# onecodex/finch-rs

Hardware: AMD Instinct MI355X
Metric: bases/sec sketched (k=21, n=1000) (higher is better)
Workload: dtype u64; 1 GPU; 50.0 Gbase synthetic 150 bp reads in total (BASELINE configs[3]), split into 1 contiguous read block (one per GPU), mash k=21 n=1000 seed 0, blocks resident in HBM as packed stream, partial sketches merged on the host; reads_per_gpu=333333334, reads_total=333333334, parallelism=read-block sharding x1, host merge; one process, one GPU

## Files before the change

finch_rs_amd/csrc/build.py:

```python
#!/usr/bin/env python3
import os
import subprocess
import sys
from concurrent.futures import ThreadPoolExecutor

HERE = os.path.dirname(os.path.abspath(__file__))
PKG = os.path.dirname(HERE)
OUT = os.path.join(PKG, "libfinch_hip.so")
OBJ = os.path.join(HERE, "obj")
NPARTS = 4
HIPCC = os.environ.get("HIPCC", "/opt/rocm/bin/hipcc")
FLAGS = ["--offload-arch=gfx950", "-O3", "-std=c++17", "-fPIC", "-Wall", "-Wno-unused-function", "-Wno-cuda-compat"]
FLAGS += os.environ.get("FH_EXTRA_FLAGS", "").split()
K2_FLAGS = ["-mllvm", "-amdgpu-sched-strategy=max-ilp", "-mllvm", "-pragma-unroll-threshold=200000"]
if "FH_K2_FLAGS" in os.environ:
    K2_FLAGS = os.environ["FH_K2_FLAGS"].split()
K2S_FLAGS_LAST = ["-mllvm", "-amdgpu-sched-strategy=iterative-ilp", "-mllvm", "-pragma-unroll-threshold=200000"]
if "FH_K2S_FLAGS_LAST" in os.environ:
    K2S_FLAGS_LAST = os.environ["FH_K2S_FLAGS_LAST"].split()
elif "FH_K2_FLAGS" in os.environ:
    K2S_FLAGS_LAST = K2_FLAGS
if "FH_OUT" in os.environ:
    OUT = os.environ["FH_OUT"]
    OBJ = os.path.join(HERE, "obj", "ab_" + os.path.splitext(os.path.basename(OUT))[0])

K2WS_FLAGS = os.environ["FH_K2WS_FLAGS"].split() if "FH_K2WS_FLAGS" in os.environ else ["-mllvm", "-amdgpu-sched-strategy=max-ilp"]
K2W_FLAGS = os.environ["FH_K2W_FLAGS"].split() if "FH_K2W_FLAGS" in os.environ else ["-mllvm", "-amdgpu-sched-strategy=max-ilp"]
SOURCES = ["fh_core.h", "fh_device.h", "fh_kernels.h", "fh_k2_common.h", "fh_k2_lds.h", "fh_internal.h", "fh_options.h", "fh_options.cpp", "fh_k2b.hip", "fh_k2bw.hip", "fh_batch.hip", "fh_batch_plan.h", "fh_batch_large.hip", "fh_records.hip", "fh_records_plan.h", "fh_screen.hip", "fh_screen.h", "fh_epilogue_dev.h", "fh_k2w.hip", "fh_k2.hip", "fh_k2s.hip", "fh_k2ws.hip", "fh_kernels.hip", "fh_big.hip", "fh_text.hip", "fh_bgzf.hip", "fh_api.hip", "fh_dist.hip", "fh_dist.h", "fh_dist_dev.h", "fh_index.hip", "fh_index.h", "fh_cluster.h", "fh_merge_path.h", "fh_gather.hip", "fh_matrix.hip", "fh_matrix.h", "fh_moments.hip", "fh_moments.h", "fh_merge_lib.hip", "fh_merge_lib.h", "fh_counts.hip", "fh_counts.h", "fh_host.cpp", "fh_library.cpp",
           "fh_host_model.h", "fh_inflate.h", "fh_pargz.h", "fh_slot_pipe.h", "fh_entries.h", "fh_serial.cpp", os.path.join("..", "..", "include", "finch_host.h"),
           os.path.join("..", "..", "include", "finch_hip.h")]


def _newest_src():
    return max(os.path.getmtime(os.path.join(HERE, s)) for s in SOURCES)


def _run(cmd):
    r = subprocess.run(cmd, cwd=HERE, stdout=subprocess.PIPE, stderr=subprocess.STDOUT, text=True)
    if r.returncode != 0:
        raise RuntimeError("command failed: %s\n%s" % (" ".join(cmd), r.stdout))
    return r.stdout


# ... 90 lines not shown
```

finch_rs_amd/csrc/fh_api.hip:

```cpp
#include <hip/hip_runtime.h>
#include <sched.h>

#include <algorithm>
#include <atomic>
#include <chrono>
#include <cmath>
#include <cstdarg>
#include <cstdio>
#include <cstdlib>
#include <cstring>
#include <condition_variable>
#include <mutex>
#include <string>
#include <thread>
#include <vector>

#include "../../include/finch_hip.h"
#include "fh_core.h"
#include "fh_counts.h"
#include "fh_strip.h"
#include "fh_device.h"
#include "fh_kernels.h"
#include "fh_internal.h"
#include "fh_options.h"

using namespace fh;

namespace {

thread_local std::string g_err;

int fail(int code, const char *fmt, ...) {
    char buf[512];
    va_list ap;
    va_start(ap, fmt);
    vsnprintf(buf, sizeof buf, fmt, ap);
    va_end(ap);
    g_err = buf;
    return code;
// ... 116 lines not shown
    } spec;
    uint64_t n_fast_finish = 0, n_spec_deferred = 0, n_spec_recovered = 0;
    uint32_t epi_pending = 0, epi_units = 0;
    uint8_t *proc_buf = nullptr;
    uint64_t proc_cap = 0, proc_fill = 0, proc_total_bases = 0;
    bool proc_continuing = false, proc_in_record = false, proc_in_cut = false;
    bool device_clean = false;
    uint64_t final_text_bases = 0;
    uint32_t *left_buf[2] = {nullptr, nullptr};
    uint32_t seg_hint = 0, blk_seg = 0, blk_sub = 1;
    uint64_t gran = TILE_POS;
    uint32_t *h_probe = nullptr;
    bool probe_seen = false;
    hipEvent_t probe_ev = nullptr;
    uint32_t probe_answer = 0;
    uint32_t probe_breakers = 0;
    uint64_t n_seg_launches = 0, n_seg_probes = 0;
    uint64_t max_waves = 0;
    uint64_t max_range = 0;
    uint64_t tau_lo = 0;
    bool no_spec = false;
    uint64_t n_spec = 0, n_spec_fallback = 0, n_spec_rescaled = 0;
    uint32_t *smp_list = nullptr, *smp_hist = nullptr, *h_smp_hist = nullptr;
    uint64_t smp_list_cap = 0;
    uint64_t n_sampled = 0;
    uint64_t ins_seen = 0;
    double novelty = 1.0;
    uint64_t n_launches = 0, n_relaunches = 0;
    uint8_t *h_stage[N_STAGE] = {nullptr, nullptr};
    uint8_t *d_stage[N_STAGE] = {nullptr, nullptr};
// ... 207 lines not shown
    if (s->open_loop) {
        P = ((remaining + G - 1) / G) * G;
    } else {
        const double room = (double)s->live_target - (double)std::min<uint64_t>(s->last_live, s->live_target);
        const double fr = fill_rate(s);
        double p = fr > 0.0 ? (s->big_mode ? 1.0 : 0.5) * room / fr : 1e19;
        P = p >= 1e18 ? remaining + G : (uint64_t)p;
    }
    if (s->max_range) P = std::min<uint64_t>(P, s->max_range);
    P = std::max<uint64_t>((P / G) * G, G);
    return std::min<uint64_t>(P, ((remaining + G - 1) / G) * G);
}

int check_ctl(fh_sketcher *s);
int flush_epilogue(fh_sketcher *s);
int recover_spec(fh_sketcher *s);
int reread_above(fh_sketcher *s, const uint8_t *seq, uint64_t len, uint64_t base_pos, uint64_t p_begin, uint64_t p_end, uint64_t lo);
int sketch_positions(fh_sketcher *s, const uint8_t *d_seq, uint64_t len, uint64_t base_pos, uint64_t pos, uint64_t n_pos, uint64_t lo_end);
int big_prune(fh_sketcher *s, bool sorted = true);
int grow_table(fh_sketcher *s, uint64_t new_live_cap);

int collect_profile(fh_sketcher *s) {
    for (size_t i = 0; i < s->prof_used; ++i) {
        float ms = 0.f;
        HIP_TRY(hipEventElapsedTime(&ms, s->prof_events[i].first, s->prof_events[i].second));
        s->prof_ms += ms;
    }
    s->prof_used = 0;
    return FH_OK;
}
// ... 161 lines not shown
    r.seq = d_seq;
    r.len = len;
    r.base_pos = base_pos;
    r.p_begin = pos;
    r.p_end = end;
    r.seg = (s->blk_seg && (s->p.k > 32 || (!s->p.hash_mask && !s->tau_lo)) && pos % s->gran == 0) ? s->blk_seg : 0u;
    r.seg_sub = r.seg ? s->blk_sub : 1u;
    const uint64_t tile = r.seg ? (uint64_t)seg_tile_pos(r.seg, r.seg_sub) : (uint64_t)TILE_POS;
    const uint64_t tiles = (end - pos + tile - 1) / tile;
    if (tiles >= (1ull << 31)) return fail(FH_ERR_INVALID, "block too large for one range");
    r.tiles_total = (uint32_t)tiles;
    static const uint32_t unit_knob = [] {
        const char *e = cfg("unit_tiles");
        return e ? (uint32_t)atoi(e) : 0u;
    }();
    r.unit_tiles = unit_knob ? unit_knob : (tiles < (uint64_t)UNIT_TILES * 2 * s->max_waves ? 1u : (uint32_t)UNIT_TILES);
    r.max_units = MAX_UNITS;
    if (r.seg) {
        static const uint32_t seg_pull = [] {
            const char *e = cfg("seg_pull_pos");
            return e ? (uint32_t)atoi(e) : (uint32_t)MAX_UNITS * UNIT_TILES * TILE_POS;
        }();
        if (!unit_knob) r.unit_tiles = 1u;
        r.max_units = std::max<uint32_t>(1u, seg_pull / (uint32_t)(tile * r.unit_tiles));
    }
    r.n_units = (uint32_t)((tiles + r.unit_tiles - 1) / r.unit_tiles);
    r.n_left_in = 0;
    r.left_cur = 0;
    r.gated = gated;
    r.verdict = spec_tau != 0;
    r.admit_at_start = admit_rate(s->last_tau);
// ... 11 lines not shown
    HIP_TRY(launch_queue_reset(s->ctl, 1u, soft_limit_of(s), read_first_of(s), s->stream, spec_tau != 0, spec_tau, gated, first_total));
    if (int rc = launch_pending(s)) return rc;
    r.active = true;
    if (s->profiling) s->prof_positions += end - pos;
    s->dirty = true;
    return FH_OK;
}

int set_tau(fh_sketcher *s, uint64_t tau) {
    if (int rc = flush_epilogue(s)) return rc;
    HIP_TRY(launch_set_tau(s->ctl, tau, s->stream));
    s->last_tau = tau;
    return FH_OK;
}

constexpr uint64_t SPEC_MAX_POS = 64ull << 20, SPEC_PREFIX_POS = 32ull << 20;
int speculative_first_block(fh_sketcher *s, const uint8_t *d_seq, uint64_t len, uint64_t base_pos, uint64_t n_pos,
                            bool *done) {
    *done = false;
    const double want = 4.0 * (double)std::max<uint64_t>(s->p.size, 1);
    if (s->no_spec || s->max_range || s->p.hash_mask || n_pos < 32768 || n_pos > SPEC_MAX_POS ||
        want * 2.0 >= (double)n_pos)
        return FH_OK;
    if (s->p.kind == FH_KIND_SCALED && s->p.size == 0) return FH_OK;
    uint64_t tau_spec = (uint64_t)(want / (double)n_pos * 18446744073709551616.0);
    if (s->p.kind == FH_KIND_SCALED) tau_spec = std::max(tau_spec, s->max_hash);
    if (tau_spec == 0 || tau_spec >= EMPTY64 - 1) return FH_OK;
    if (s->fast && !s->big_mode && s->p.kind == FH_KIND_MASH && s->p.size > 0) {
        s->n_spec++;
        s->n_spec_deferred++;
        const bool was_open = s->open_loop;
// ... 222 lines not shown
            s->prof_used++;
        }
        HIP_TRY(launch_ac_count((int)s->p.k, a, s->stream));
        if (e1) {
            HIP_TRY(hipEventRecord(e1, s->stream));
            s->prof_launches++;
            s->prof_positions += a.p_end - a.p_begin;
        }
        s->n_launches++;
    }
    s->positions_done += n_pos;
    s->ac_dirty = true;
    return FH_OK;
}

int sketch_device_range(fh_sketcher *s, const uint8_t *d_seq, uint64_t len, uint64_t base_pos) {
    if (int rc = drain(s)) return rc;
    if (len < s->p.k) return FH_OK;
    if (s->p.kind == FH_KIND_ALL_COUNTS) return ac_count_block(s, d_seq, len);
    const uint64_t n_pos = len - s->p.k + 1;
    s->blk_seg = 0;
    s->blk_sub = 1;
    s->gran = TILE_POS;
    bool probe_behind = false;
    {
        static const bool seg_off = cfg("no_seg") != nullptr;
        static const uint64_t probe_min = [] {
            const char *e = cfg("seg_probe_min");
            return e ? strtoull(e, nullptr, 10) : (16ull << 20);
        }();
        static const uint64_t probe_wait_min = [] {
// ... 45 lines not shown
    struct ProbeBehind {
        fh_sketcher *s;
        const uint8_t *seq;
        uint64_t len;
        bool on;
        ~ProbeBehind() {
            if (!on || !s->h_probe) return;
            if (launch_seg_probe(seq, len, s->h_probe, s->stream) == hipSuccess) {
                if (!s->probe_ev && hipEventCreateWithFlags(&s->probe_ev, hipEventDisableTiming) != hipSuccess) s->probe_ev = nullptr;
                if (s->probe_ev) (void)hipEventRecord(s->probe_ev, s->stream);
                s->probe_seen = true;
                s->n_seg_probes++;
            }
        }
    } probe_guard{s, d_seq, len, probe_behind};
    uint64_t pos = 0;
    uint64_t lo_end = 0;
    bool sampled = false;
    if (s->positions_done == 0 && s->tau_lo == 0) {
        bool done = false;
        if (int rc = sampled_first_block(s, d_seq, len, base_pos, n_pos, &sampled, &done)) return rc;
        if (sampled && done) return FH_OK;
        if (sampled) lo_end = n_pos;
    }
    if (!sampled && s->positions_done == 0 && s->tau_lo == 0) {
        static const uint64_t prefix_pos = cfg("spec_prefix_pos") ? std::max<uint64_t>(1ull << 20, strtoull(cfg("spec_prefix_pos"), nullptr, 10)) : SPEC_PREFIX_POS;
        const uint64_t spec_pos = n_pos <= SPEC_MAX_POS ? n_pos : std::max<uint64_t>(prefix_pos / s->gran, 1) * s->gran;
        bool done = false;
        if (int rc = speculative_first_block(s, d_seq, len, base_pos, spec_pos, &done)) return rc;
        if (done) {
            if (spec_pos == n_pos) return FH_OK;
            pos = spec_pos;
        } else if (s->tau_lo) {
            if (int rc = reread_above(s, d_seq, len, base_pos, 0, spec_pos, s->tau_lo)) return rc;
            if (spec_pos == n_pos) return FH_OK;
            pos = spec_pos;
        }
    }
    return sketch_positions(s, d_seq, len, base_pos, pos, n_pos, lo_end);
}

int sketch_positions(fh_sketcher *s, const uint8_t *d_seq, uint64_t len, uint64_t base_pos, uint64_t pos, uint64_t n_pos, uint64_t lo_end) {
// ... 78 lines not shown
    if ((uint64_t)s->last_live >= s->p.size) {
        s->positions_done += sp.n_pos;
    } else {
        s->n_spec_fallback++;
        if (int rc = reread_above(s, sp.range.seq, sp.range.len, sp.range.base_pos, sp.range.p_begin, sp.range.p_end, sp.tau)) return rc;
    }
    if (queued.active)
        if (int rc = sketch_positions(s, queued.seq, queued.len, queued.base_pos, queued.p_begin, queued.p_end, 0)) return rc;
    return FH_OK;
}

int check_ctl(fh_sketcher *s) {
    if (int rc = flush_epilogue(s)) return rc;
    HIP_TRY(hipMemcpyAsync(s->h_ctl, s->ctl, sizeof(Ctl), hipMemcpyDeviceToHost, s->stream));
    HIP_TRY(hipStreamSynchronize(s->stream));
    if (s->h_ctl->overflow == 1) return fail(FH_ERR_CAPACITY, "device hash table capacity exceeded");
    if (s->h_ctl->overflow == 2) return fail(FH_ERR_CAPACITY, "hash collision log capacity exceeded");
    return FH_OK;
}

int ensure_big_buffers(fh_sketcher *s, uint32_t M) {
    if (M <= s->big_cap) return FH_OK;
    HIP_TRY(hipStreamSynchronize(s->stream));
    if (s->keys_a) { (void)hipFree(s->keys_a); (void)hipFree(s->keys_b); (void)hipFree(s->slots_a); (void)hipFree(s->slots_b); (void)hipFree(s->sort_tmp); }
    s->keys_a = s->keys_b = nullptr; s->slots_a = s->slots_b = nullptr; s->sort_tmp = nullptr;
    const uint32_t cap = (uint32_t)std::min<uint64_t>((uint64_t)M + M / 2 + 1024, s->live_cap);
    HIP_TRY(dev_malloc(&s->keys_a, (size_t)cap * 8));
    HIP_TRY(dev_malloc(&s->keys_b, (size_t)cap * 8));
    HIP_TRY(dev_malloc(&s->slots_a, (size_t)cap * 4));
    HIP_TRY(dev_malloc(&s->slots_b, (size_t)cap * 4));
// ... 491 lines not shown
        uint64_t held = handle_bytes(s);
        for (const fh_sketcher *q : g_pool) held += handle_bytes(q);
        if (g_pool.size() < pool_max() && held <= pool_max_bytes()) {
            g_pool.push_back(s);
            return;
        }
    }
    destroy_handle(s);
}

namespace {
void destroy_handle(fh_sketcher *s) {
    if (!s) return;
    (void)hipSetDevice(s->device);
    if (s->stream) (void)hipStreamSynchronize(s->stream);
    for (auto &pe : s->prof_events) {
        (void)hipEventDestroy(pe.first);
        (void)hipEventDestroy(pe.second);
    }
    for (int i = 0; i < N_STAGE; ++i) {
        if (s->h_stage[i]) (void)hipHostFree(s->h_stage[i]);
        if (s->d_stage[i]) (void)hipFree(s->d_stage[i]);
        if (s->stage_done[i]) (void)hipEventDestroy(s->stage_done[i]);
        (void)hipFree(s->d_packed[i]);
        (void)hipFree(s->d_blk_a[i]);
        (void)hipFree(s->d_blk_b[i]);
    }
    (void)hipFree(s->d_text_tot);
    (void)hipFree(s->d_lines);
    for (int q = 0; q < fh_sketcher::BZ_STREAMS; ++q) {
// ... 52 lines not shown
    if (s->h_smp_hist) (void)hipHostFree(s->h_smp_hist);
    if (s->h_probe) (void)hipHostFree(s->h_probe);
    if (s->probe_ev) (void)hipEventDestroy(s->probe_ev);
    if (s->copy_stream) {
        (void)hipStreamSynchronize(s->copy_stream);
        (void)hipStreamDestroy(s->copy_stream);
    }
    if (s->stream) (void)hipStreamDestroy(s->stream);
    delete s;
}
}

int fh_reset(fh_sketcher *s) {
    if (!s) return fail(FH_ERR_INVALID, "null handle");
    if (int rc = set_device(s)) return rc;
    gzip_quiesce(s);
    if (s->ac_table && (s->ac_dirty || s->ac_check)) {
        const uint64_t bins = ac_bins((int)s->p.k);
        HIP_TRY(hipMemsetAsync(s->ac_table, 0, bins * 4, s->stream));
        HIP_TRY(hipMemsetAsync(s->ac_sat, 0, std::max<uint64_t>(bins / 8, 4), s->stream));
    }
    s->ac_dirty = s->ac_check = false;
    s->ac_windows = 0;
    if (s->device_clean && s->finished && !s->pend.active && !s->epi_pending) {
        s->device_clean = false;
        return init_state(s, false);
    }
    s->device_clean = false;
    if (s->spec.pending && !s->pend.active) s->spec.pending = false;
    if (int rc = drain(s)) return rc;
// ... 129 lines not shown
    if (!s) return fail(FH_ERR_INVALID, "null argument");
    if (launches) *launches = s->n_seg_launches;
    if (probes) *probes = s->n_seg_probes;
    if (stride) *stride = s->blk_seg;
    return FH_OK;
}

int fh_push_device(fh_sketcher *s, const void *dev_bytes, uint64_t len) {
    if (!s || (!dev_bytes && len)) return fail(FH_ERR_INVALID, "null argument");
    if (s->finished) return fail(FH_ERR_STATE, "sketcher already finished; call fh_reset");
    if (int rc = proc_flush(s)) return rc;
    if (((uintptr_t)dev_bytes & 15u) != 0) return fail(FH_ERR_INVALID, "device block must be 16-byte aligned");
    if (int rc = set_device(s)) return rc;
    s->carry_len = 0;
    s->dprev_len = 0;
    int rc = sketch_device_range(s, (const uint8_t *)dev_bytes, len, s->stream_off);
    s->stream_off += len;
    return rc;
}

static uint64_t strip_block(uint8_t *dst, const uint8_t *src, uint64_t n) {
    static const unsigned cap = [] {
        const char *e = cfg("host_threads");
        const unsigned v = e ? (unsigned)atoi(e) : 8u;
        return v ? v : 1u;
    }();
    const unsigned hw = std::max(1u, std::thread::hardware_concurrency());
    const size_t nt = std::min<size_t>(std::min<size_t>(hw, cap), n >> 21);
    if (nt <= 1) return fh_strip::strip(dst, src, n);
    const size_t per = (n + nt - 1) / nt;
    std::vector<size_t> kept(nt + 1, 0);
    auto lo_of = [&](size_t t) { return std::min<size_t>(n, t * per); };
// ... 729 lines not shown
        *total_bases = s->final_text_bases;
        return FH_OK;
    }
    if (int rc = set_device(s)) return rc;
    if (int rc = drain(s)) return rc;
    if (int rc = check_ctl(s)) return rc;
    *total_bases = s->h_ctl->text_bases;
    return FH_OK;
}

int fh_push_block(fh_sketcher *s, const uint8_t *bytes, uint64_t len) { return fh_push_block_ex(s, bytes, len, 0u); }

int fh_sync(fh_sketcher *s) {
    if (!s) return fail(FH_ERR_INVALID, "null handle");
    if (int rc = set_device(s)) return rc;
    if (int rc = proc_flush(s)) return rc;
    if (int rc = drain(s)) return rc;
    if (int rc = check_ctl(s)) return rc;
    return collect_profile(s);
}

static size_t result_count(const fh_sketcher *s) { return s->res_built ? s->res.size() : s->r_n; }

static int ensure_wide(fh_sketcher *s) {
    if (!s->wide_pending) return FH_OK;
    if (int rc = set_device(s)) return rc;
    const size_t n = s->r_n;
    HIP_TRY(hipMemcpyAsync(s->r_hash, s->o_hash, n * 8ull, hipMemcpyDeviceToHost, s->stream));
    HIP_TRY(hipMemcpyAsync(s->r_kmer, s->o_kmer, n * 8ull, hipMemcpyDeviceToHost, s->stream));
    if (s->r_kmer_hi) HIP_TRY(hipMemcpyAsync(s->r_kmer_hi, s->o_kmer_hi, n * 8ull, hipMemcpyDeviceToHost, s->stream));
// ... 73 lines not shown
        HIP_TRY(dev_malloc(&tmp, bytes));
        HIP_TRY(hipMemcpyPeerAsync(tmp, dst->device, src->ac_table, src->device, bytes, dst->stream));
        from = tmp;
    }
    hipError_t e = launch_ac_add(dst->ac_table, from, ac_bins((int)dst->p.k), dst->stream);
    if (e == hipSuccess) e = hipStreamSynchronize(dst->stream);
    (void)hipFree(tmp);
    if (e != hipSuccess) return fail(FH_ERR_HIP, "fh_merge (AllCounts): %s", hipGetErrorString(e));
    dst->ac_check = dst->ac_dirty = true;
    return ac_finish(dst);
}

int fh_finish(fh_sketcher *s, uint64_t *n_out, uint64_t *total_kmers) {
    if (!s) return fail(FH_ERR_INVALID, "null handle");
    if (int rc = set_device(s)) return rc;
    if (s->p.kind == FH_KIND_ALL_COUNTS) {
        if (!s->finished) {
            if (int rc = proc_flush(s)) return rc;
            if (int rc = ac_finish(s)) return rc;
        }
        if (n_out) *n_out = s->r_n;
        if (total_kmers) *total_kmers = s->total_kmers;
        return FH_OK;
    }
    static const bool trace = cfg("trace") != nullptr;
    auto now = [] { return std::chrono::steady_clock::now(); };
    auto ms = [](std::chrono::steady_clock::time_point a, std::chrono::steady_clock::time_point b) {
        return std::chrono::duration<double, std::milli>(b - a).count();
    };
    const auto t0 = now();
// ... 16 lines not shown
            if (int rc = ensure_out(s, (uint32_t)std::min<uint64_t>(s->p.size + 1, SMALL_MAX))) return rc;
            if (int rc = ensure_h_out(s->out_stride * (wide ? 40 : 32) + 64)) return rc;
            static const bool no_fold = cfg("no_reset_fold") != nullptr;
            EpiArgs e = epi_args(s, s->epi_pending | EPI_PRUNE_FORCE | EPI_SORT | EPI_GATHER | (s->spec.pending ? EPI_NEED_SPEC : 0u) |
                                        (no_fold ? 0u : EPI_RESET));
            e.n_units = s->epi_units;
            s->epi_pending = 0;
            e.check_units = s->pend.active ? s->pend.n_units : 0u;
            e.tau0 = initial_tau(s);
            e.hist_on = s->hist ? 1u : 0u;
            e.out = (uint64_t *)s->h_out;
            e.out_stride = (uint32_t)s->out_stride;
            e.h_ctl = s->h_ctl;
            HIP_TRY(launch_small_epilogue(e, s->stream));
            HIP_TRY(hipStreamSynchronize(s->stream));
            const Ctl &c = *s->h_ctl;
            if (c.overflow == 1) return fail(FH_ERR_CAPACITY, "device hash table capacity exceeded");
            if (c.overflow == 2) return fail(FH_ERR_CAPACITY, "hash collision log capacity exceeded");
            fused = c.sorted == FIN_OK || c.sorted == FIN_OK_RESET;
            s->device_clean = c.sorted == FIN_OK_RESET;
            if (fused) {
                s->spec.pending = false;
                s->pend.active = false;
                s->last_tau = c.tau;
                s->last_live = c.n_live;
                s->ins_seen = c.inserted_total;
                s->n_fast_finish++;
            }
        }
        if (!fused) {
// ... 702 lines not shown
```

finch_rs_amd/csrc/fh_kernels.hip:

```cpp
#include <hip/hip_runtime.h>

#include <atomic>

#include "fh_core.h"
#include "fh_device.h"
#include "fh_epilogue_dev.h"
#include "fh_kernels.h"

namespace fh {

hipError_t launch_k2(int k, const SketchArgs &a, int blocks, hipStream_t st) {
    static_assert(FH_NPARTS == 4, "dispatcher below is written for 4 parts");
    if (k < 1 || k > FH_MAX_K) return hipErrorInvalidValue;
    if (k > 32 && a.seg_stride) {
        if (!seg_launch_ok((uint32_t)k, a.seg_stride, a.seg_sub)) return hipErrorInvalidValue;
        switch ((k - 33) / (32 / FH_NPARTS)) {
        case 0: return launch_k2ws_part0(k, a, st);
        case 1: return launch_k2ws_part1(k, a, st);
        case 2: return launch_k2ws_part2(k, a, st);
        default: return launch_k2ws_part3(k, a, st);
        }
    }
    if (k > 32) {
        switch ((k - 33) / (32 / FH_NPARTS)) {
// ... 140 lines not shown
        const u64 key = keys[i];
        if (((u32)(key >> shift) & 2047u) == bin) list[atomicAdd(&wsum[0], 1u)] = key;
    }
    __syncthreads();
    const u32 want = rank - below - 1u;
    if (tid < in_bin) {
        const u64 mine = list[tid];
        u32 smaller = 0;
        for (u32 j = 0; j < in_bin; ++j) smaller += list[j] < mine ? 1u : 0u;
        if (smaller == want) bcast[0] = mine;
    }
    __syncthreads();
    const u64 r = bcast[0];
    __syncthreads();
    return r;
}

struct SmallLds {
    u64 *keys;
    u64 *skeys;
    u32 *sslots;
    u32 *hist;
    u32 *wsum;
    u64 *bcast;
    u32 *cnt;
};
constexpr size_t SMALL_LDS_BYTES = (size_t)SMALL_MAX * 8 + (size_t)SMALL_SORT_MAX * 12;
constexpr u32 PRUNE_DECLINED = 0xFFFFFFFFu;

__device__ __forceinline__ void sort_wide_dev(u32 *live, u32 *scratch, u32 M, const SmallLds L) {
// ... 45 lines not shown
    u64 *keys = L.keys;
    constexpr int PER = SMALL_MAX / 1024;
    u32 my_slot[PER];
#pragma unroll
    for (int j = 0; j < PER; ++j) {
        const u32 i = tid + (u32)j * 1024u;
        my_slot[j] = 0u;
        if (i < M) {
            const u32 sl = live[i];
            my_slot[j] = sl;
            keys[i] = table[sl].hash;
        }
    }
    if (tid < 2) L.cnt[tid] = 0;
    __syncthreads();
    u64 tau;
    u32 keep;
    if (kind == 0u) {
        if ((u64)M >= size && size > 0) {
            tau = lds_select_kth_fast(keys, M, (u32)size, L.hist, L.wsum, L.bcast, reinterpret_cast<unsigned char *>(L.skeys));
            keep = (u32)size;
        } else if (size == 0) {
            tau = 0ull;
            keep = 0;
        } else {
            tau = EMPTY64;
            keep = M;
        }
    } else {
        u32 c = 0;
// ... 19 lines not shown
    if (sort_out && keep > (u32)SMALL_SORT_MAX) {
        const u32 nd_now = ctl->n_dead;
        if (!keep_all || keep != M || nd_now > dead_cap || M > dead_cap - nd_now) {
            if (tid == 0) ctl->need_big = 1u;
            return PRUNE_DECLINED;
        }
        sort_wide_dev(live, dead + nd_now, M, L);
        if (tid == 0) {
            ctl->n_live = keep;
            const u64 cur = ctl->tau;
            ctl->tau = tau < cur ? tau : cur;
            ctl->sorted = 1u;
        }
        return keep;
    }
    const u32 nd0 = ctl->n_dead;
    const u32 ndrop = M - keep;
    const bool dead_fits = nd0 != 0xFFFFFFFFu && nd0 <= dead_cap && ndrop <= dead_cap - nd0;
    const bool none = size == 0 && kind == 0u;
    if (keep < M || sort_out) {
#pragma unroll
        for (int j = 0; j < PER; ++j) {
            const u32 i = tid + (u32)j * 1024u;
            if (i < M) {
                const u64 key = keys[i];
                const bool k = none ? false : (keep == M || key <= tau);
                if (k) {
                    const u32 pos = atomicAdd(&L.cnt[0], 1u);
                    if (sort_out) {
                        L.skeys[pos] = key;
                        L.sslots[pos] = my_slot[j];
                    } else {
                        live[pos] = my_slot[j];
                    }
                } else if (dead_fits) {
                    dead[nd0 + atomicAdd(&L.cnt[1], 1u)] = my_slot[j];
                }
            }
        }
    }
    __syncthreads();
    if (sort_out && keep <= 1024u) {
        u64 key = tid < keep ? L.skeys[tid] : EMPTY64;
        u32 slot = tid < keep ? L.sslots[tid] : 0xFFFFFFFFu;
        for (u32 kk = 2; kk <= 1024u; kk <<= 1) {
            for (u32 jj = kk >> 1; jj > 0; jj >>= 1) {
                u64 pk;
                u32 ps;
                if (jj >= 64u) {
                    __syncthreads();
                    L.skeys[tid] = key;
                    L.sslots[tid] = slot;
                    __syncthreads();
                    pk = L.skeys[tid ^ jj];
                    ps = L.sslots[tid ^ jj];
                } else {
                    pk = __shfl_xor(key, (int)jj);
                    ps = __shfl_xor(slot, (int)jj);
                }
                const bool keep_min = ((tid & kk) == 0u) == ((tid & jj) == 0u);
                if (keep_min ? (pk < key) : (pk > key)) {
                    key = pk;
                    slot = ps;
                }
            }
        }
        __syncthreads();
        L.skeys[tid] = key;
        L.sslots[tid] = slot;
        __syncthreads();
        if (tid < keep) live[tid] = slot;
    } else if (sort_out) {
        u32 N = 1;
        while (N < keep) N <<= 1;
        for (u32 i = keep + tid; i < N; i += nthr) {
            L.skeys[i] = EMPTY64;
            L.sslots[i] = 0xFFFFFFFFu;
        }
        __syncthreads();
        bitonic_lds(L.skeys, L.sslots, N);
        for (u32 i = tid; i < keep; i += nthr) live[i] = L.sslots[i];
    }
    if (tid == 0) {
        ctl->n_live = keep;
        const u64 cur = ctl->tau;
        ctl->tau = tau < cur ? tau : cur;
        ctl->sorted = sort_out ? 1u : 0u;
        ctl->n_dead = dead_fits ? nd0 + ndrop : 0xFFFFFFFFu;
    }
    return keep;
}

__device__ __forceinline__ SmallLds small_lds(unsigned char *smem, u32 *hist, u32 *wsum, u64 *bcast, u32 *cnt) {
    SmallLds L;
    L.keys = reinterpret_cast<u64 *>(smem);
    L.skeys = reinterpret_cast<u64 *>(smem + (size_t)SMALL_MAX * 8);
    L.sslots = reinterpret_cast<u32 *>(smem + (size_t)SMALL_MAX * 8 + (size_t)SMALL_SORT_MAX * 8);
// ... 38 lines not shown
    return hipSuccess;
}

hipError_t launch_prune_small(Entry *table, u32 *live, u32 *dead, u32 dead_cap, Ctl *ctl, u32 kind, u64 size,
                              u64 max_hash, u32 trigger, u32 force, u32 sort_out, hipStream_t st) {
    if (hipError_t e = small_lds_attr(reinterpret_cast<const void *>(k3_prune_small)); e != hipSuccess) return e;
    hipLaunchKernelGGL(k3_prune_small, dim3(1), dim3(1024), SMALL_LDS_BYTES, st, table, live, dead, dead_cap, ctl, kind, size,
                       max_hash, trigger, force, sort_out);
    return hipGetLastError();
}

__device__ __forceinline__ u32 small_epilogue_body(const EpiArgs &a, unsigned char *smem, u32 *s_hist, u32 *s_wsum, u64 *s_bcast,
                                                   u32 *s_cnt, u32 *s_off, u32 &s_live) {
    Ctl *ctl = a.ctl;
    const u32 tid = threadIdx.x, lane = tid & 63u, wave = tid >> 6;
    const bool skip = (a.flags & EPI_GATED) && ctl->spec_ok == 0u;
    if (!skip) {
        u32 M = ctl->n_live;
        if (a.flags & EPI_FLATTEN) {
            static_assert(N_SHARDS == 256, "the scan below is written for 256 shards");
            u32 c = 0;
            if (tid < (u32)N_SHARDS) {
                c = ctl->shard_cnt[tid * SHARD_STRIDE];
                if (c > ctl->shard_cap) c = ctl->shard_cap;
            }
            u32 inc = c;
            for (int off = 1; off < 64; off <<= 1) {
                const u32 t = __shfl_up(inc, off);
                if (lane >= (u32)off) inc += t;
            }
// ... 23 lines not shown
            }
            if (tid < (u32)N_SHARDS) ctl->shard_cnt[tid * SHARD_STRIDE] = 0;
            if (tid == 0 && total) {
                ctl->inserted_total += total;
                u32 n = M + total;
                if (n > live_cap) n = live_cap;
                ctl->n_live = n;
                ctl->sorted = 0;
                s_live = n;
            } else if (tid == 0) {
                s_live = M;
            }
            __syncthreads();
            M = s_live;
        }
        u32 kept = PRUNE_DECLINED;
        const u32 force = a.flags & EPI_PRUNE_FORCE, sort_out = (a.flags & EPI_SORT) ? 1u : 0u;
        if ((a.flags & (EPI_PRUNE_FORCE | EPI_PRUNE_TRIGGER)) && !ctl->need_big && (force || M > a.trigger)) {
            if (M > (u32)SMALL_MAX) {
                if (tid == 0) ctl->need_big = 1u;
            } else {
                kept = prune_small_dev(a.table, a.live, a.dead, a.dead_cap, ctl, M, a.kind, a.size, a.max_hash, sort_out,
                                       small_lds(smem, s_hist, s_wsum, s_bcast, s_cnt), a.flags & EPI_KEEP_ALL);
            }
        }
        __syncthreads();
        if (a.flags & EPI_VERDICT) {
            if (tid == 0) {
                const bool dry = ctl->next_unit >= a.n_units && ctl->n_left_out == 0u;
                const bool ok = dry && kept != PRUNE_DECLINED && (u64)kept >= a.size && !ctl->need_big && !ctl->overflow;
                ctl->spec_ok = ok ? 1u : 0u;
            }
        }
        if ((a.flags & EPI_GATHER) && kept != PRUNE_DECLINED) {
            const SmallLds L = small_lds(smem, s_hist, s_wsum, s_bcast, s_cnt);
            const size_t st = a.out_stride;
            u64 *o_hash = a.out, *o_kmer = o_hash + st, *o_pos = o_kmer + st;
            u64 *o_kmer_hi = a.wide ? o_pos + st : nullptr;
            u32 *o_count = (u32 *)((a.wide ? o_kmer_hi : o_pos) + st), *o_extra = o_count + st;
            const bool from_live = kept > (u32)SMALL_SORT_MAX;
            for (u32 i = tid; i < kept; i += 1024u) {
                const u32 sl = from_live ? a.live[i] : L.sslots[i];
                const Entry e = a.table[sl];
                o_hash[i] = from_live ? e.hash : L.skeys[i];
                const u64 occ = e.count + e.extra;
                o_count[i] = occ > 0xFFFFFFFFull ? 0xFFFFFFFFu : (u32)occ;
                o_extra[i] = e.extra > 0xFFFFFFFFull ? 0xFFFFFFFFu : (u32)e.extra;
                o_kmer[i] = e.kmer;
                if (o_kmer_hi) o_kmer_hi[i] = ctl->kmer_hi[sl];
                o_pos[i] = e.pos;
            }
        }
    }
    u32 fin = 0u;
    if ((a.flags & EPI_GATHER) && !skip) {
        __syncthreads();
        const bool spec_ok = !(a.flags & EPI_NEED_SPEC) || ctl->spec_ok != 0u;
        const bool dry = a.check_units == 0u || (ctl->next_unit >= a.check_units && ctl->n_left_out == 0u);
        const bool rows_ok = (a.flags & EPI_KEEP_ALL) ? true : (u64)ctl->n_live <= a.size;
        const bool ok = spec_ok && dry && !ctl->need_big && !ctl->overflow && ctl->sorted == 1u && rows_ok;
        if (ok) fin = ((a.flags & EPI_RESET) && ctl->n_dead != 0xFFFFFFFFu) ? FIN_OK_RESET : FIN_OK;
        __syncthreads();
        if (fin && tid == 0) ctl->sorted = fin;
    }
    if (a.h_ctl) {
        __syncthreads();
        const u32 *src = reinterpret_cast<const u32 *>(ctl);
        u32 *dst = reinterpret_cast<u32 *>(a.h_ctl);
        for (u32 i = tid; i < (u32)(sizeof(Ctl) / 4); i += 1024u) dst[i] = src[i];
        __threadfence_system();
    }
    if (fin == FIN_OK_RESET) {
        __syncthreads();
        const SmallLds L = small_lds(smem, s_hist, s_wsum, s_bcast, s_cnt);
        const u32 nl = ctl->n_live, nd = ctl->n_dead;
        u64 *khi = ctl->kmer_hi;
        const bool from_live = nl > (u32)SMALL_SORT_MAX;
        for (u32 i = tid; i < nl; i += 1024u) {
            const u32 sl = from_live ? a.live[i] : L.sslots[i];
            clear_entry(&a.table[sl]);
            if (khi) khi[sl] = EMPTY64;
        }
        for (u32 i = tid; i < nd; i += 1024u) {
            const u32 sl = a.dead[i];
            clear_entry(&a.table[sl]);
            if (khi) khi[sl] = EMPTY64;
        }
        __syncthreads();
        init_ctl_dev(ctl, a.tau0, 0u, a.size, (a.flags & EPI_KEEP_ALL) ? a.max_hash : 0ull, a.hist_on);
    }
    return fin;
}

__global__ __launch_bounds__(1024) void k_small_epilogue(const EpiArgs a) {
    extern __shared__ __attribute__((aligned(16))) unsigned char smem[];
    __shared__ u32 s_hist[256];
    __shared__ u32 s_wsum[16];
    __shared__ u64 s_bcast[2];
    __shared__ u32 s_cnt[2];
    __shared__ u32 s_off[N_SHARDS + 1];
    __shared__ u32 s_live;
    (void)small_epilogue_body(a, smem, s_hist, s_wsum, s_bcast, s_cnt, s_off, s_live);
}

__global__ __launch_bounds__(1024) void k_batch_epilogue(const EpiArgs *args, u32 read_first) {
// ... 448 lines not shown
```

Before: 775.1 billion bases/s.

## Run segment probe on side stream, round spec prefix to full waves, speed epilogue sort/clear

For caller-resident device blocks, the segment probe now launches on a separate non-blocking stream and is joined at sync, finish, reset and error points, so it overlaps with the main sketch instead of trailing it. The speculative prefix length is rounded so its tiles fill whole waves of the grid. The 1024-element epilogue sort now does wave-local bitonic sorts followed by a rank merge through binary search, which avoids the LDS-synchronised cross-wave stages. Table reset clears entries word by word to coalesce stores. Optional timestamp instrumentation is added behind a compile flag. The cost is extra stream and event management and added join points.

```diff
diff --git a/finch_rs_amd/csrc/build.py b/finch_rs_amd/csrc/build.py
--- a/finch_rs_amd/csrc/build.py
+++ b/finch_rs_amd/csrc/build.py
@@ -26,7 +26,7 @@
 
 K2WS_FLAGS = os.environ["FH_K2WS_FLAGS"].split() if "FH_K2WS_FLAGS" in os.environ else ["-mllvm", "-amdgpu-sched-strategy=max-ilp"]
 K2W_FLAGS = os.environ["FH_K2W_FLAGS"].split() if "FH_K2W_FLAGS" in os.environ else ["-mllvm", "-amdgpu-sched-strategy=max-ilp"]
-SOURCES = ["fh_core.h", "fh_device.h", "fh_kernels.h", "fh_k2_common.h", "fh_k2_lds.h", "fh_internal.h", "fh_options.h", "fh_options.cpp", "fh_k2b.hip", "fh_k2bw.hip", "fh_batch.hip", "fh_batch_plan.h", "fh_batch_large.hip", "fh_records.hip", "fh_records_plan.h", "fh_screen.hip", "fh_screen.h", "fh_epilogue_dev.h", "fh_k2w.hip", "fh_k2.hip", "fh_k2s.hip", "fh_k2ws.hip", "fh_kernels.hip", "fh_big.hip", "fh_text.hip", "fh_bgzf.hip", "fh_api.hip", "fh_dist.hip", "fh_dist.h", "fh_dist_dev.h", "fh_index.hip", "fh_index.h", "fh_cluster.h", "fh_merge_path.h", "fh_gather.hip", "fh_matrix.hip", "fh_matrix.h", "fh_moments.hip", "fh_moments.h", "fh_merge_lib.hip", "fh_merge_lib.h", "fh_counts.hip", "fh_counts.h", "fh_host.cpp", "fh_library.cpp",
+SOURCES = ["fh_core.h", "fh_device.h", "fh_kernels.h", "fh_k2_common.h", "fh_k2_lds.h", "fh_internal.h", "fh_options.h", "fh_spec_plan.h", "fh_options.cpp", "fh_k2b.hip", "fh_k2bw.hip", "fh_batch.hip", "fh_batch_plan.h", "fh_batch_large.hip", "fh_records.hip", "fh_records_plan.h", "fh_screen.hip", "fh_screen.h", "fh_epilogue_dev.h", "fh_k2w.hip", "fh_k2.hip", "fh_k2s.hip", "fh_k2ws.hip", "fh_kernels.hip", "fh_big.hip", "fh_text.hip", "fh_bgzf.hip", "fh_api.hip", "fh_dist.hip", "fh_dist.h", "fh_dist_dev.h", "fh_index.hip", "fh_index.h", "fh_cluster.h", "fh_merge_path.h", "fh_gather.hip", "fh_matrix.hip", "fh_matrix.h", "fh_moments.hip", "fh_moments.h", "fh_merge_lib.hip", "fh_merge_lib.h", "fh_counts.hip", "fh_counts.h", "fh_host.cpp", "fh_library.cpp",
            "fh_host_model.h", "fh_inflate.h", "fh_pargz.h", "fh_slot_pipe.h", "fh_entries.h", "fh_serial.cpp", os.path.join("..", "..", "include", "finch_host.h"),
            os.path.join("..", "..", "include", "finch_hip.h")]
 
diff --git a/finch_rs_amd/csrc/fh_api.hip b/finch_rs_amd/csrc/fh_api.hip
--- a/finch_rs_amd/csrc/fh_api.hip
+++ b/finch_rs_amd/csrc/fh_api.hip
@@ -23,6 +23,7 @@
 #include "fh_kernels.h"
 #include "fh_internal.h"
 #include "fh_options.h"
+#include "fh_spec_plan.h"
 
 using namespace fh;
 
@@ -169,6 +170,8 @@
     bool probe_seen = false;
     hipEvent_t probe_ev = nullptr;
     uint32_t probe_answer = 0;
+    hipStream_t probe_stream = nullptr;
+    bool probe_out = false;
     uint32_t probe_breakers = 0;
     uint64_t n_seg_launches = 0, n_seg_probes = 0;
     uint64_t max_waves = 0;
@@ -406,6 +409,30 @@
 
 int check_ctl(fh_sketcher *s);
 int flush_epilogue(fh_sketcher *s);
+
+bool probe_beside(fh_sketcher *s, const uint8_t *seq, uint64_t len) {
+    if (!s->probe_stream && hipStreamCreateWithFlags(&s->probe_stream, hipStreamNonBlocking) != hipSuccess) s->probe_stream = nullptr;
+    if (!s->probe_ev && hipEventCreateWithFlags(&s->probe_ev, hipEventDisableTiming) != hipSuccess) s->probe_ev = nullptr;
+    if (!s->probe_stream || !s->probe_ev) {
+        (void)hipGetLastError();
+        return false;
+    }
+    if (launch_seg_probe(seq, len, s->h_probe, s->probe_stream) != hipSuccess) return false;
+    s->probe_out = true;
+    (void)hipEventRecord(s->probe_ev, s->probe_stream);
+    s->probe_seen = true;
+    s->n_seg_probes++;
+    return true;
+}
+void probe_join(fh_sketcher *s) {
+    if (!s->probe_out) return;
+    if (hipEventSynchronize(s->probe_ev) != hipSuccess) (void)hipStreamSynchronize(s->probe_stream);
+    s->probe_out = false;
+}
+struct ProbeJoinOnExit {
+    fh_sketcher *s;
+    ~ProbeJoinOnExit() { probe_join(s); }
+};
 int recover_spec(fh_sketcher *s);
 int reread_above(fh_sketcher *s, const uint8_t *seq, uint64_t len, uint64_t base_pos, uint64_t p_begin, uint64_t p_end, uint64_t lo);
 int sketch_positions(fh_sketcher *s, const uint8_t *d_seq, uint64_t len, uint64_t base_pos, uint64_t pos, uint64_t n_pos, uint64_t lo_end);
@@ -597,7 +624,7 @@
         const char *e = cfg("unit_tiles");
         return e ? (uint32_t)atoi(e) : 0u;
     }();
-    r.unit_tiles = unit_knob ? unit_knob : (tiles < (uint64_t)UNIT_TILES * 2 * s->max_waves ? 1u : (uint32_t)UNIT_TILES);
+    r.unit_tiles = unit_knob ? unit_knob : fh_spec::tile_unit_tiles(tiles, s->max_waves);
     r.max_units = MAX_UNITS;
     if (r.seg) {
         static const uint32_t seg_pull = [] {
@@ -639,7 +666,9 @@
     return FH_OK;
 }
 
-constexpr uint64_t SPEC_MAX_POS = 64ull << 20, SPEC_PREFIX_POS = 32ull << 20;
+using fh_spec::SPEC_MAX_POS;
+using fh_spec::SPEC_PREFIX_POS;
+static_assert(fh_spec::TILE_POS == (uint64_t)TILE_POS && fh_spec::UNIT_TILES == (uint32_t)UNIT_TILES, "fh_spec_plan.h restates fh_device.h");
 int speculative_first_block(fh_sketcher *s, const uint8_t *d_seq, uint64_t len, uint64_t base_pos, uint64_t n_pos,
                             bool *done) {
     *done = false;
@@ -892,7 +921,7 @@
     return FH_OK;
 }
 
-int sketch_device_range(fh_sketcher *s, const uint8_t *d_seq, uint64_t len, uint64_t base_pos) {
+int sketch_device_range(fh_sketcher *s, const uint8_t *d_seq, uint64_t len, uint64_t base_pos, bool callers_block = false) {
     if (int rc = drain(s)) return rc;
     if (len < s->p.k) return FH_OK;
     if (s->p.kind == FH_KIND_ALL_COUNTS) return ac_count_block(s, d_seq, len);
@@ -968,6 +997,7 @@
             }
         }
     } probe_guard{s, d_seq, len, probe_behind};
+    if (probe_behind && callers_block && s->h_probe && probe_beside(s, d_seq, len)) probe_guard.on = false;
     uint64_t pos = 0;
     uint64_t lo_end = 0;
     bool sampled = false;
@@ -978,8 +1008,9 @@
         if (sampled) lo_end = n_pos;
     }
     if (!sampled && s->positions_done == 0 && s->tau_lo == 0) {
-        static const uint64_t prefix_pos = cfg("spec_prefix_pos") ? std::max<uint64_t>(1ull << 20, strtoull(cfg("spec_prefix_pos"), nullptr, 10)) : SPEC_PREFIX_POS;
-        const uint64_t spec_pos = n_pos <= SPEC_MAX_POS ? n_pos : std::max<uint64_t>(prefix_pos / s->gran, 1) * s->gran;
+        static const uint64_t prefix_pos = cfg("spec_prefix_pos") ? std::max<uint64_t>(fh_spec::SPEC_PREFIX_MIN, strtoull(cfg("spec_prefix_pos"), nullptr, 10)) : SPEC_PREFIX_POS;
+        const uint64_t wpb = s->blk_seg ? (uint64_t)seg_waves_per_block((int)s->p.k) : (uint64_t)k2_waves_per_block((int)s->p.k);
+        const uint64_t spec_pos = n_pos <= SPEC_MAX_POS ? n_pos : fh_spec::prefix_positions(prefix_pos, s->gran, s->blk_seg != 0, s->max_waves, wpb);
         bool done = false;
         if (int rc = speculative_first_block(s, d_seq, len, base_pos, spec_pos, &done)) return rc;
         if (done) {
@@ -1088,6 +1119,7 @@
     if (int rc = flush_epilogue(s)) return rc;
     HIP_TRY(hipMemcpyAsync(s->h_ctl, s->ctl, sizeof(Ctl), hipMemcpyDeviceToHost, s->stream));
     HIP_TRY(hipStreamSynchronize(s->stream));
+    probe_join(s);
     if (s->h_ctl->overflow == 1) return fail(FH_ERR_CAPACITY, "device hash table capacity exceeded");
     if (s->h_ctl->overflow == 2) return fail(FH_ERR_CAPACITY, "hash collision log capacity exceeded");
     return FH_OK;
@@ -1609,6 +1641,10 @@
     if (!s) return;
     (void)hipSetDevice(s->device);
     if (s->stream) (void)hipStreamSynchronize(s->stream);
+    if (s->probe_stream) {
+        (void)hipStreamSynchronize(s->probe_stream);
+        (void)hipStreamDestroy(s->probe_stream);
+    }
     for (auto &pe : s->prof_events) {
         (void)hipEventDestroy(pe.first);
         (void)hipEventDestroy(pe.second);
@@ -1691,6 +1727,7 @@
 int fh_reset(fh_sketcher *s) {
     if (!s) return fail(FH_ERR_INVALID, "null handle");
     if (int rc = set_device(s)) return rc;
+    probe_join(s);
     gzip_quiesce(s);
     if (s->ac_table && (s->ac_dirty || s->ac_check)) {
         const uint64_t bins = ac_bins((int)s->p.k);
@@ -1850,8 +1887,9 @@
     if (int rc = set_device(s)) return rc;
     s->carry_len = 0;
     s->dprev_len = 0;
-    int rc = sketch_device_range(s, (const uint8_t *)dev_bytes, len, s->stream_off);
+    int rc = sketch_device_range(s, (const uint8_t *)dev_bytes, len, s->stream_off, true);
     s->stream_off += len;
+    if (rc != FH_OK) probe_join(s);
     return rc;
 }
 
@@ -2611,6 +2649,7 @@
 int fh_sync(fh_sketcher *s) {
     if (!s) return fail(FH_ERR_INVALID, "null handle");
     if (int rc = set_device(s)) return rc;
+    ProbeJoinOnExit probe_joined{s};
     if (int rc = proc_flush(s)) return rc;
     if (int rc = drain(s)) return rc;
     if (int rc = check_ctl(s)) return rc;
@@ -2714,6 +2753,7 @@
 int fh_finish(fh_sketcher *s, uint64_t *n_out, uint64_t *total_kmers) {
     if (!s) return fail(FH_ERR_INVALID, "null handle");
     if (int rc = set_device(s)) return rc;
+    ProbeJoinOnExit probe_joined{s};
     if (s->p.kind == FH_KIND_ALL_COUNTS) {
         if (!s->finished) {
             if (int rc = proc_flush(s)) return rc;
@@ -2760,6 +2800,7 @@
             e.h_ctl = s->h_ctl;
             HIP_TRY(launch_small_epilogue(e, s->stream));
             HIP_TRY(hipStreamSynchronize(s->stream));
+            probe_join(s);
             const Ctl &c = *s->h_ctl;
             if (c.overflow == 1) return fail(FH_ERR_CAPACITY, "device hash table capacity exceeded");
             if (c.overflow == 2) return fail(FH_ERR_CAPACITY, "hash collision log capacity exceeded");
diff --git a/finch_rs_amd/csrc/fh_kernels.hip b/finch_rs_amd/csrc/fh_kernels.hip
--- a/finch_rs_amd/csrc/fh_kernels.hip
+++ b/finch_rs_amd/csrc/fh_kernels.hip
@@ -178,6 +178,35 @@
     const u64 r = bcast[0];
     __syncthreads();
     return r;
+}
+
+#ifdef FH_EPI_STAMPS
+__device__ u64 g_epi_stamps[16];
+#define EPI_STAMP(i)                                                                  \
+    do {                                                                              \
+        if (threadIdx.x == 0 && blockIdx.x == 0) g_epi_stamps[i] = wall_clock64();    \
+    } while (0)
+extern "C" int fh_debug_epi_stamps(unsigned long long *out16) {
+    return (int)hipMemcpyFromSymbol(out16, HIP_SYMBOL(g_epi_stamps), sizeof(u64) * 16);
+}
+#else
+#define EPI_STAMP(i) \
+    do {             \
+    } while (0)
+#endif
+
+template <class SlotAt>
+__device__ __forceinline__ void clear_entries_by_word(Entry *table, u32 n, u64 *khi, SlotAt slot_at) {
+    static_assert(sizeof(Entry) == 40 && offsetof(Entry, hash) == 0 && offsetof(Entry, kmer) == 8 && offsetof(Entry, pos) == 16 &&
+                      offsetof(Entry, count) == 24 && offsetof(Entry, extra) == 32,
+                  "three words of EMPTY64, then the two counters");
+    const u32 words = n * 5u;
+    for (u32 w = threadIdx.x; w < words; w += blockDim.x) {
+        const u32 e = w / 5u, f = w - e * 5u;
+        const u32 sl = slot_at(e);
+        reinterpret_cast<u64 *>(&table[sl])[f] = f < 3u ? EMPTY64 : 0ull;
+        if (khi && f == 0u) khi[sl] = EMPTY64;
+    }
 }
 
 struct SmallLds {
@@ -253,6 +282,7 @@
     }
     if (tid < 2) L.cnt[tid] = 0;
     __syncthreads();
+    EPI_STAMP(2);
     u64 tau;
     u32 keep;
     if (kind == 0u) {
@@ -302,6 +332,7 @@
         }
         return keep;
     }
+    EPI_STAMP(3);
     const u32 nd0 = ctl->n_dead;
     const u32 ndrop = M - keep;
     const bool dead_fits = nd0 != 0xFFFFFFFFu && nd0 <= dead_cap && ndrop <= dead_cap - nd0;
@@ -328,25 +359,16 @@
         }
     }
     __syncthreads();
+    EPI_STAMP(4);
     if (sort_out && keep <= 1024u) {
         u64 key = tid < keep ? L.skeys[tid] : EMPTY64;
         u32 slot = tid < keep ? L.sslots[tid] : 0xFFFFFFFFu;
-        for (u32 kk = 2; kk <= 1024u; kk <<= 1) {
+        const u32 lane = tid & 63u;
+        for (u32 kk = 2; kk <= 64u; kk <<= 1) {
             for (u32 jj = kk >> 1; jj > 0; jj >>= 1) {
-                u64 pk;
-                u32 ps;
-                if (jj >= 64u) {
-                    __syncthreads();
-                    L.skeys[tid] = key;
-                    L.sslots[tid] = slot;
-                    __syncthreads();
-                    pk = L.skeys[tid ^ jj];
-                    ps = L.sslots[tid ^ jj];
-                } else {
-                    pk = __shfl_xor(key, (int)jj);
-                    ps = __shfl_xor(slot, (int)jj);
-                }
-                const bool keep_min = ((tid & kk) == 0u) == ((tid & jj) == 0u);
+                const u64 pk = __shfl_xor(key, (int)jj);
+                const u32 ps = __shfl_xor(slot, (int)jj);
+                const bool keep_min = ((lane & kk) == 0u) == ((lane & jj) == 0u);
                 if (keep_min ? (pk < key) : (pk > key)) {
                     key = pk;
                     slot = ps;
@@ -355,9 +377,26 @@
         }
         __syncthreads();
         L.skeys[tid] = key;
-        L.sslots[tid] = slot;
-        __syncthreads();
-        if (tid < keep) live[tid] = slot;
+        __syncthreads();
+        u32 cnt[16];
+#pragma unroll
+        for (int o = 0; o < 16; ++o) cnt[o] = 0u;
+#pragma unroll
+        for (u32 step = 32u; step > 0u; step >>= 1) {
+#pragma unroll
+            for (int o = 0; o < 16; ++o)
+                if (L.skeys[(u32)o * 64u + cnt[o] + step - 1u] < key) cnt[o] += step;
+        }
+        u32 rank = 0u;
+#pragma unroll
+        for (int o = 0; o < 16; ++o) rank += cnt[o] + (L.skeys[(u32)o * 64u + cnt[o]] < key ? 1u : 0u);
+        __syncthreads();
+        if (key != EMPTY64) {
+            L.skeys[rank] = key;
+            L.sslots[rank] = slot;
+            live[rank] = slot;
+        }
+        __syncthreads();
     } else if (sort_out) {
         u32 N = 1;
         while (N < keep) N <<= 1;
@@ -369,6 +408,7 @@
         bitonic_lds(L.skeys, L.sslots, N);
         for (u32 i = tid; i < keep; i += nthr) live[i] = L.sslots[i];
     }
+    EPI_STAMP(5);
     if (tid == 0) {
         ctl->n_live = keep;
         const u64 cur = ctl->tau;
@@ -437,6 +477,7 @@
                                                    u32 *s_cnt, u32 *s_off, u32 &s_live) {
     Ctl *ctl = a.ctl;
     const u32 tid = threadIdx.x, lane = tid & 63u, wave = tid >> 6;
+    EPI_STAMP(0);
     const bool skip = (a.flags & EPI_GATED) && ctl->spec_ok == 0u;
     if (!skip) {
         u32 M = ctl->n_live;
@@ -490,6 +531,10 @@
             __syncthreads();
             M = s_live;
         }
+        EPI_STAMP(1);
+#ifdef FH_EPI_STAMPS
+        if (tid == 0 && blockIdx.x == 0) g_epi_stamps[12] = M;
+#endif
         u32 kept = PRUNE_DECLINED;
         const u32 force = a.flags & EPI_PRUNE_FORCE, sort_out = (a.flags & EPI_SORT) ? 1u : 0u;
         if ((a.flags & (EPI_PRUNE_FORCE | EPI_PRUNE_TRIGGER)) && !ctl->need_big && (force || M > a.trigger)) {
@@ -501,6 +546,7 @@
             }
         }
         __syncthreads();
+        EPI_STAMP(6);
         if (a.flags & EPI_VERDICT) {
             if (tid == 0) {
                 const bool dry = ctl->next_unit >= a.n_units && ctl->n_left_out == 0u;
@@ -531,6 +577,7 @@
     u32 fin = 0u;
     if ((a.flags & EPI_GATHER) && !skip) {
         __syncthreads();
+        EPI_STAMP(7);
         const bool spec_ok = !(a.flags & EPI_NEED_SPEC) || ctl->spec_ok != 0u;
         const bool dry = a.check_units == 0u || (ctl->next_unit >= a.check_units && ctl->n_left_out == 0u);
         const bool rows_ok = (a.flags & EPI_KEEP_ALL) ? true : (u64)ctl->n_live <= a.size;
@@ -539,6 +586,7 @@
         __syncthreads();
         if (fin && tid == 0) ctl->sorted = fin;
     }
+    EPI_STAMP(8);
     if (a.h_ctl) {
         __syncthreads();
         const u32 *src = reinterpret_cast<const u32 *>(ctl);
@@ -546,25 +594,24 @@
         for (u32 i = tid; i < (u32)(sizeof(Ctl) / 4); i += 1024u) dst[i] = src[i];
         __threadfence_system();
     }
+    EPI_STAMP(9);
     if (fin == FIN_OK_RESET) {
         __syncthreads();
         const SmallLds L = small_lds(smem, s_hist, s_wsum, s_bcast, s_cnt);
         const u32 nl = ctl->n_live, nd = ctl->n_dead;
         u64 *khi = ctl->kmer_hi;
         const bool from_live = nl > (u32)SMALL_SORT_MAX;
-        for (u32 i = tid; i < nl; i += 1024u) {
-            const u32 sl = from_live ? a.live[i] : L.sslots[i];
-            clear_entry(&a.table[sl]);
-            if (khi) khi[sl] = EMPTY64;
-        }
-        for (u32 i = tid; i < nd; i += 1024u) {
-            const u32 sl = a.dead[i];
-            clear_entry(&a.table[sl]);
-            if (khi) khi[sl] = EMPTY64;
-        }
-        __syncthreads();
+#ifdef FH_EPI_STAMPS
+        if (tid == 0 && blockIdx.x == 0) g_epi_stamps[13] = nl, g_epi_stamps[14] = nd;
+#endif
+        const u32 *const live_list = a.live, *const dead_list = a.dead, *const sorted_slots = L.sslots;
+        clear_entries_by_word(a.table, nl, khi, [=](u32 i) { return from_live ? live_list[i] : sorted_slots[i]; });
+        clear_entries_by_word(a.table, nd, khi, [=](u32 i) { return dead_list[i]; });
+        __syncthreads();
+        EPI_STAMP(10);
         init_ctl_dev(ctl, a.tau0, 0u, a.size, (a.flags & EPI_KEEP_ALL) ? a.max_hash : 0ull, a.hist_on);
     }
+    EPI_STAMP(11);
     return fin;
 }
 
diff --git a/finch_rs_amd/csrc/fh_spec_plan.h b/finch_rs_amd/csrc/fh_spec_plan.h
--- /dev/null
+++ b/finch_rs_amd/csrc/fh_spec_plan.h
@@ -0,0 +1,30 @@
+#pragma once
+#include <cstdint>
+
+namespace fh_spec {
+
+constexpr uint64_t TILE_POS = 2048;
+constexpr uint32_t UNIT_TILES = 2;
+constexpr uint64_t SPEC_MAX_POS = 64ull << 20, SPEC_PREFIX_POS = 32ull << 20, SPEC_PREFIX_MIN = 1ull << 20;
+
+constexpr uint32_t tile_unit_tiles(uint64_t tiles, uint64_t max_waves) { return tiles < (uint64_t)UNIT_TILES * 2 * max_waves ? 1u : UNIT_TILES; }
+
+constexpr uint64_t grid_waves(uint64_t units, uint64_t max_waves, uint64_t wpb) {
+    const uint64_t w = units < 1 ? 1 : (units < max_waves ? units : max_waves);
+    return (w + wpb - 1) / wpb * wpb;
+}
+
+constexpr uint64_t prefix_positions(uint64_t want, uint64_t tile, bool seg, uint64_t max_waves, uint64_t wpb) {
+    const uint64_t tiles_down = want / tile < 1 ? 1 : want / tile;
+    if (max_waves == 0 || wpb == 0 || max_waves % wpb != 0) return tiles_down * tile;
+    uint64_t tiles = (want + tile - 1) / tile;
+    for (int pass = 0; pass < 2; ++pass) {
+        const uint64_t ut = seg ? 1u : tile_unit_tiles(tiles, max_waves);
+        const uint64_t units = (tiles + ut - 1) / ut;
+        const uint64_t waves = 2 * units > max_waves ? max_waves : grid_waves(units, max_waves, wpb);
+        tiles = (units + waves - 1) / waves * waves * ut;
+    }
+    return tiles * tile <= SPEC_MAX_POS ? tiles * tile : tiles_down * tile;
+}
+
+}
```

After: 775.9 billion bases/s (median of 6 runs). No clear change (+0.1%).
